# lordet01/SE_SNMF_NAT

Measured on AMD Instinct MI355X. Metric: NMF multiplicative-update iterations/sec (FxTxr), higher is better.
Workload: dtype f32; 1 GPU; single-MI355X sparse NMF basis train (BASELINE configs[1]): 257x100000 frames, r=256, KL, sparsity=5.0, full W+H update + objective per step; F=257, T=100000, r=256, beta=1, settle_steps=150

## Files before the change

### se_snmf_nat_amd/csrc/snmf_internal.h

```cpp
#pragma once
#include "snmf_kernels.h"

#include <algorithm>
#include <cmath>
#include <cstdarg>
#include <cstdio>
#include <cstring>
#include <deque>
#include <map>
#include <mutex>
#include <string>
#include <vector>

#include "snmf.h"

using namespace snmf;

extern thread_local std::string g_err;
int fail(int code, const char* fmt, ...);
#define HIP_TRY(expr)                                                                              \
    do {                                                                                           \
        hipError_t e_ = (expr);                                                                    \
        if (e_ != hipSuccess)                                                                      \
            return fail(e_ == hipErrorOutOfMemory ? SNMF_ERR_NOMEM : SNMF_ERR_NO_DEVICE, "%s: %s", \
// ... 82 lines not shown
    int NKT = 8, NWB = 4, WPS = 2, NLW = 0;
    int nbw = 2;
    int n_fg = 1, n_kg = 1, n_chunks = 1;
    static constexpr int stagger_w = 0;
    bool sf = false;
    int sf_grid = 1;
    bool wsf = false;
    size_t lds_wsf = 0;
    bool isf_share = false;
    bool wsf_share = false;
    bool isf = false;
    size_t lds_isf = 0;
    static constexpr int sf_stagger = 8000;
    size_t lds_sf = 0;
    int sf_share = 0, sf_nfull = 0;
    bool sr = false, wsr = false;
    int sr_grid = 1;
    static constexpr int sr_stagger = 1300;
    size_t lds_sr = 0, lds_wsr = 0;
    int til = 1;
    int n_ch1 = 0;
    bool wxg_off = false;
    bool wxg = false;
    int kq_chunks = 0, kq_kg = 0;
    size_t kq_lds = 0;
    size_t lds_w = 0;
    bool wfin = false;
    int wfin_S = 1;
    size_t lds_wfin = 0;
    bool fold_obj = false;
    bool gram_p = false;
    int gram_chunks = 0;
    bool generic = false;
    int frame_fb = 0, frame_kb = 0;
    size_t lds_frame = 0;
    size_t lds_mdi = 0;
    int grid_mdi = 1;
    bool small = false;
    bool small_ok = false;
    size_t lds_small = 0;
};
int plan_geometry(const snmf_params* p, int n_cu, PlanGeometry* g);
void describe_geometry(const PlanGeometry& g, const snmf_params& p, int n_cu, bool mdi, char* buf, size_t n);

struct snmf_plan : PlanGeometry {
    snmf_ctx* ctx = nullptr;
// ... 117 lines not shown
```

### se_snmf_nat_amd/csrc/snmf_kernels.h

```cpp
#pragma once
#include <hip/hip_runtime.h>
#include <stdint.h>

namespace snmf {

typedef float f32x2 __attribute__((ext_vector_type(2)));

typedef float f32x16 __attribute__((ext_vector_type(16)));
typedef float f32x4 __attribute__((ext_vector_type(4)));

constexpr float kFlr = 1e-9f;
constexpr int kMaxNW = 12;

constexpr int BM_GEN = 0;
constexpr int BM_KL = 1;
constexpr int BM_EUC = 2;

__device__ __forceinline__ f32x16 mfma32(float a, float b, f32x16 c) {
    return __builtin_amdgcn_mfma_f32_32x32x2f32(a, b, c, 0, 0, 0);
}
__device__ __forceinline__ f32x16 zero16() {
    f32x16 z;
#pragma unroll
    for (int i = 0; i < 16; ++i) z[i] = 0.f;
// ... 321 lines not shown
        wA[0] = ldw(q + 4);
        wA[1] = ldw(q + 5);
        sA[0] = *reinterpret_cast<const f32x4*>(bp + 32);
        sA[1] = *reinterpret_cast<const f32x4*>(bp + 40);
        bp += 32;
        SNMF_PIN();
        mmstage(wB, sB);
    }
    if (q < nq) {
#pragma unroll
        for (int e = 0; e < 4; ++e) acc = mfma32(sA[0][e], wA[0][e], acc);
    }
    if (q + 1 < nq) {
#pragma unroll
        for (int e = 0; e < 4; ++e) acc = mfma32(sA[1][e], wA[1][e], acc);
    }
    if (q + 2 < nq) {
        const f32x4 w2 = ldw(q + 2);
        const f32x4 s2 = *reinterpret_cast<const f32x4*>(bp + 16);
#pragma unroll
        for (int e = 0; e < 4; ++e) acc = mfma32(s2[e], w2[e], acc);
    }
}

__device__ __forceinline__ void stagger_start(int cycles, unsigned linear_block, unsigned n_blocks, int shift) {
    const bool late = shift >= 0 ? ((linear_block >> shift) & 1u) != 0 : linear_block >= n_blocks / 2;
    if (cycles > 0 && late) {
        const unsigned long long t0 = __builtin_amdgcn_s_memtime();
        while (__builtin_amdgcn_s_memtime() - t0 < (unsigned long long)cycles) __builtin_amdgcn_s_sleep(32);
    }
}

template <int NTHREADS>
__device__ __forceinline__ void stage_in(const float* __restrict__ src, float* dst, int cols, int rowlen, int ld,
                                         int tid) {
    const int r4 = rowlen / 4;
    const int n4 = cols * r4;
    constexpr int B = 8;
    for (int i0 = tid; i0 < n4; i0 += B * NTHREADS) {
        f32x4 x[B];
#pragma unroll
        for (int b = 0; b < B; ++b) {
            const int i = i0 + b * NTHREADS;
            if (i < n4) x[b] = *reinterpret_cast<const f32x4*>(src + 4 * (size_t)i);
        }
        SNMF_PIN();
// ... 2359 lines not shown
            dps[k] = k < sa.Rx ? 0.f : hw;
        }
        __builtin_amdgcn_wave_barrier();
        for (int part = 0; part < 2; ++part) {
            hsolve_frame_p1<FB, KB>(wr, part ? dps : sps, wxs, lamp, xlam, Fm, xr, kb, fb, lane);
            __syncthreads();
            for (int f = tid; f < Fm && f < F; f += NTHR) {
                float s = lamp[f];
#pragma unroll
                for (int q = 1; q < 8; ++q) s += lamp[q * Fm + f];
                out[part * F + f] = s;
            }
            if (xr && tid == 0) {
                float s = xlam[0];
#pragma unroll
                for (int q = 1; q < 8; ++q) s += xlam[q];
                out[part * F + Fm] = s;
            }
            __syncthreads();
        }
    }
}

template <int NK, int NWB, int NL, int WPS, int WM, int BM, bool OBJ, int TT, int LX, bool TIL, bool XG = false>
__device__ __forceinline__ void wstats_body(StepArgs a, int n_chunks, int mat_index, int n_mat) {
    static_assert(TT == 32 || (TT == 16 && NL == 0), "narrow tiles: 16 frames, synchronous staging");
    static_assert(!XG || (WM != 3 && !TIL), "the extra row rides in P3's gate: needs a P3, every consumer on every tile");
    constexpr int NTHR = (NWB + NL) * 64;
    const int NBUF = NL > 0 ? (a.nbuf == 3 ? 3 : 2) : 1;
    if (a.stop && *a.stop) return;
    extern __shared__ __attribute__((aligned(16))) float lds[];
    const int ldv = 32 * NWB;
    constexpr bool LDHC = (NK == 4 || NK == 8) && TT == 32;
    const int ldh = LDHC ? (NK == 4 ? 132 : 260) : a.ldh;
    const int bufsz = TT * (ldh + ldv);
    float* wxs = lds + NBUF * bufsz;
    const int lane = threadIdx.x & 63, w = wave_index();
    const bool is_loader = NL > 0 && w >= NWB;
    const int fl = lane & 31, h = lane >> 5;
    const int rp = a.rp, Fp = a.Fp;
    int chunk = blockIdx.x, by = blockIdx.y, nch = n_chunks;
    if (a.n_ch1 > 0) {
        by = 0;
        if (chunk >= n_chunks) {
            const int c1 = chunk - n_chunks;
            by = 1 + c1 / a.n_ch1;
            chunk = c1 - (by - 1) * a.n_ch1;
            nch = a.n_ch1;
        }
    }
// ... 38 lines not shown
    const bool do_s = WM == 0 && by == 0 && blockIdx.z == 0;
    float ssum[4] = {0.f, 0.f, 0.f, 0.f};
    double acc_div = 0.0;

    static_assert(NL == 0 || (NL == 4 && (NWB == 4 || NWB == 8)), "progress slots: four per loader role, NWB consumers");
    unsigned* ready = reinterpret_cast<unsigned*>(wxs + rp);
    unsigned* done = ready + 4;
    float* vx = reinterpret_cast<float*>(done + NWB);
    float* gxs = wxs + rp + 128;
    const unsigned gxa = (unsigned)(uintptr_t)(__attribute__((address_space(3))) void*)(gxs + w * gxw + 4 * lane);
    const bool idle_c = NL > 0 && NWB == 4 && !is_loader && !active && !do_x;
    if (NL > 0) {
        if (threadIdx.x < 4 + NWB) ready[threadIdx.x] = 0u;
        __syncthreads();
        if constexpr (NWB == 4) {
            if (idle_c && lane == 0) done[w] = 0xffffffffu;
            __syncthreads();
        }
    }

    auto xrow_tile = [&](const float* xH, int xt0, int xw, const float* vxc) {
            float rxv[CPW];
            float dsum = 0.f;
#pragma unroll
            for (int c0 = 0; c0 < CPW; c0 += 4) {
                const int tl = xw * CPW + c0 + (lane >> 4);
                const int kl = lane & 15;
                const float* hrow = xH + tl * ldh;
                const int t = xt0 + tl;
                const float v = vxc[tl];
                float rv;
                if (WM != 3) {
                    float s0 = 0.f, s1 = 0.f;
                    for (int k = 4 * kl; k < rp; k += 64) {
                        const f32x4 wv = *reinterpret_cast<const f32x4*>(wxs + k);
                        const f32x4 hv = *reinterpret_cast<const f32x4*>(hrow + k);
                        s0 += wv[0] * hv[0] + wv[1] * hv[1];
                        s1 += wv[2] * hv[2] + wv[3] * hv[3];
                    }
                    const float s = row_sum_f(s0 + s1);
                    const float lam = fmaxf(s, kFlr);
                    if (OBJ && kl == 0) dsum += (t < a.T) ? div_term<BM>(v, lam, a.beta, a.inv_bb1) : 0.f;
                    if (WM == 0) rv = v * fast_rcp(lam);
                    else if (WM == 1) rv = den_of_lam<BM>(lam, a.beta);
                    else rv = v * numfac_of_lam<BM>(lam, a.beta);
                } else {
                    rv = v;
                }
#pragma unroll
                for (int c = 0; c < 4; ++c)
                    rxv[c0 + c] = __int_as_float(__builtin_amdgcn_readlane(__float_as_int(rv), 16 * c));
            }
            if (OBJ) acc_div += (double)dsum;
#pragma unroll
            for (int pc = 0; pc < NPC; ++pc) {
                const int k0 = 256 * pc + 4 * lane;
                if (k0 + (kc ? kap_base * 32 : 0) < rp) {
                    f32x4 g4;
                    if (GXL) asm volatile("ds_read_b128 %0, %1\n\ts_waitcnt lgkmcnt(0)" : "=v"(g4) : "v"(gxa));
#pragma unroll
                    for (int c = 0; c < CPW; ++c) {
                        const f32x4 hv = *reinterpret_cast<const f32x4*>(xH + (xw * CPW + c) * ldh + k0);
#pragma unroll
                        for (int e = 0; e < 4; ++e) {
                            if (GXL) g4[e] += rxv[c] * hv[e];
                            else gx[4 * pc + e] += rxv[c] * hv[e];
                        }
                    }
                    if (GXL) asm volatile("ds_write_b128 %0, %1" ::"v"(gxa), "v"(g4));
                }
            }
    };
    float rs4[NPC][4];
#pragma unroll
    for (int pp = 0; pp < NPC; ++pp)
#pragma unroll
        for (int e = 0; e < 4; ++e) rs4[pp][e] = 0.f;
    if (is_loader) {
        typedef __attribute__((address_space(3))) void* lds_ptr_t;
        const int lw = w - NWB;
        const int npc = (rp + 255) >> 8;
        const int nVb = TT * Fp * 4;
        const int c0 = by * NWB * 32;
        const int cw = (a.Fm - c0 < NWB * 32 ? a.Fm - c0 : NWB * 32);
        auto dma_tile = [&](int tile, float* dst, int bi) {
            const __amdgpu_buffer_rsrc_t rh =
                __builtin_amdgcn_make_buffer_rsrc(const_cast<float*>(a.Hin + (size_t)tile * TT * rp), 0, TT * rp * 4, 0x00020000);
            const int pc0 = kc ? (int)blockIdx.z : 0, pcn = kc ? 1 : npc;
            for (int t = lw; t < TT; t += NL)
                for (int pc = 0; pc < pcn; ++pc)
                    if ((pc0 + pc) * 256 + lane * 4 < rp)
                        __builtin_amdgcn_raw_ptr_buffer_load_lds(rh, (lds_ptr_t)(dst + t * ldh + pc * 256), 16, lane * 16,
                                                                 (t * rp + (pc0 + pc) * 256) * 4, 0, 0);
            const __amdgpu_buffer_rsrc_t rv =
                __builtin_amdgcn_make_buffer_rsrc(const_cast<float*>(a.V + (size_t)tile * TT * Fp), 0, nVb, 0x00020000);
            for (int t = lw; t < TT; t += NL)
                for (int pc = 0; pc * 256 < cw; ++pc)
                    if (pc * 256 + lane * 4 < cw)
                        __builtin_amdgcn_raw_ptr_buffer_load_lds(rv, (lds_ptr_t)(dst + TT * ldh + t * ldv + pc * 256), 16, lane * 16,
                                                                 (t * Fp + c0 + pc * 256) * 4, 0, 0);
            if (do_x && lw == 0 && lane < TT)
                __builtin_amdgcn_raw_ptr_buffer_load_lds(rv, (lds_ptr_t)(vx + bi * 32), 4, lane * Fp * 4, a.Fm * 4, 0, 0);
        };
        auto sums_of = [&](const float* H) {
            if (!do_s) return;
            for (int t = lw; t < TT; t += NL)
#pragma unroll
                for (int pc = 0; pc < NPC; ++pc)
                    if (pc < npc && pc * 256 + lane * 4 < rp) {
                        const f32x4 hv = *reinterpret_cast<const f32x4*>(H + t * ldh + pc * 256 + lane * 4);
#pragma unroll
                        for (int e = 0; e < 4; ++e) rs4[pc][e] += hv[e];
                    }
        };
        if (tb < te) {
            dma_tile(tb, lds, 0);
            asm volatile("s_waitcnt vmcnt(0)" ::: "memory");
            sums_of(lds);
            rp_post(ready, lw, 1u, lane);
        }
        int nb = 0;
        for (int tile = tb, it = 0; tile + 1 < te; ++tile, ++it) {
            nb = nb + 1 == NBUF ? 0 : nb + 1;
            float* nH = lds + nb * bufsz;
            if (it + 2 - NBUF > 0) {
                rp_await(done, (unsigned)(it + 2 - NBUF), a.stop);
                if (NWB == 8) rp_await(done + 4, (unsigned)(it + 2 - NBUF), a.stop);
            }
            dma_tile(tile + 1, nH, nb);
            asm volatile("s_waitcnt vmcnt(0)" ::: "memory");
            sums_of(nH);
            rp_post(ready, lw, (unsigned)(it + 2), lane);
        }
    }

    if (NL > 0 && NWB == 8 && !is_loader && w >= 4 && a.stagger > 0 && tb < te) {
        const unsigned long long ts = __builtin_amdgcn_s_memtime();
        while (__builtin_amdgcn_s_memtime() - ts < (unsigned long long)a.stagger) __builtin_amdgcn_s_sleep(16);
    }
    SNMF_STAMP_DECL
    int cb = NL > 0 ? NBUF - 1 : 0;
    int te_c = te;
    if constexpr (NWB == 4) {
        if (idle_c) te_c = tb;
    }
    for (int tile = tb, it = 0; tile < te_c && !is_loader; ++tile, ++it) {
        const int t0 = tile * TT;
        SNMF_STAMP(0);
        if (NL > 0) cb = cb + 1 == NBUF ? 0 : cb + 1;
        float* Hs = lds + cb * bufsz;
        float* Vs = Hs + TT * ldh;
        if (NL == 0) {
            __syncthreads();
            stage_in<NST>(a.Hin + (size_t)t0 * rp, Hs, TT, rp, ldh, sid);
            {
                const int c0 = by * NWB * 32, cw4 = (a.Fm - c0 < NWB * 32 ? a.Fm - c0 : NWB * 32) / 4, n4 = TT * cw4;
                const float* vsrc = a.V + (size_t)t0 * Fp + c0;
                constexpr int B = 8;
                for (int i0 = sid; i0 < n4; i0 += B * NST) {
                    f32x4 x[B];
#pragma unroll
                    for (int b = 0; b < B; ++b) {
                        const int i = i0 + b * NST;
                        if (i < n4) x[b] = *reinterpret_cast<const f32x4*>(vsrc + (size_t)(i / cw4) * Fp + 4 * (i % cw4));
                    }
#pragma unroll
                    for (int b = 0; b < B; ++b) {
                        const int i = i0 + b * NST;
                        if (i < n4) *reinterpret_cast<f32x4*>(Vs + (i / cw4) * ldv + 4 * (i % cw4)) = x[b];
                    }
                }
                if (do_x && sid < TT) vx[sid] = a.V[(size_t)(t0 + sid) * Fp + a.Fm];
            }
            __syncthreads();
        }
        if (NL > 0) rp_await(ready, (unsigned)(it + 1), a.stop);
        SNMF_STAMP(1);
        if (NL == 0 && do_s) {
#pragma unroll
            for (int j = 0; j < 4; ++j) {
                const int k = sid + j * NST;
                if (k < rp) {
                    float sacc = 0.f;
                    for (int t = 0; t < TT; ++t) sacc += Hs[t * ldh + k];
                    ssum[j] += sacc;
                }
            }
        }
        if (!XG && do_x) xrow_tile(Hs, t0, w, vx + cb * 32);
        SNMF_STAMP(2);
        if (!active || (TIL && til > 1 && it % til != tph)) {
            if constexpr (XG) {
                if (do_x) xrow_tile(Hs, t0, w, vx + cb * 32);
            }
            if (NL > 0) rp_post(done, w, (unsigned)(it + 1), lane);
            continue;
        }

        float R[16];
        if (WM != 3) {
            f32x16 acc1[1] = {zero16()};
            const f32x4* wp = reinterpret_cast<const f32x4*>(a.Wt4 + (size_t)phi * rp * 32) + lane;
            {
                const __amdgpu_buffer_rsrc_t rsw = wimage_rsrc(a.Wt4, (size_t)a.nf * rp * 32);
                const float* spl = Hs + (fl & (TT - 1)) * ldh + 4 * h;
                if constexpr (XG) {
                    auto xgate = [&]() {
                        if (do_x) xrow_tile(Hs, t0, w, vx + cb * 32);
                    };
                    if (a.nqk == 32) contract_p3_buf<true>(acc1[0], rsw, lane * 16, phi * rp * 128, spl, 32, xgate);
                    else contract_p3_buf<false>(acc1[0], rsw, lane * 16, phi * rp * 128, spl, a.nqk, xgate);
                } else {
                    if (a.nqk == 32) contract_p3_buf<true>(acc1[0], rsw, lane * 16, phi * rp * 128, spl, 32, NoGate());
                    else contract_p3_buf<false>(acc1[0], rsw, lane * 16, phi * rp * 128, spl, a.nqk, NoGate());
                }
            }
            SNMF_STAMP(3);
            const f32x16 acc = acc1[0];
            const int f = phi * 32 + fl;
            float dsum = 0.f;
            auto ratio_rows = [&](auto masked) {
#pragma unroll
                for (int i = 0; i < 16; ++i) {
                    if (TT < 32 && i >= TT / 2) {
                        R[i] = 0.f;
                        continue;
                    }
                    const int t = t0 + drow(i, h);
                    const float v = Vs[drow(i, h) * ldv + fc];
                    float lam = fmaxf(acc[i], kFlr);
                    if (OBJ) {
                        if (do_obj) {
                            float d = div_term<BM>(v, lam, a.beta, a.inv_bb1);
                            if (decltype(masked)::value) {
                                dsum += (f < a.F && t < a.T) ? d : 0.f;
                            } else {
#pragma clang fp contract(off)
                                dsum = dsum + d;
                            }
                        }
                    }
                    if (WM == 0) R[i] = v * fast_rcp(lam);
                    else if (WM == 1) R[i] = den_of_lam<BM>(lam, a.beta);
                    else R[i] = v * numfac_of_lam<BM>(lam, a.beta);
                }
            };
            if (OBJ && TT == 32 && phi * 32 + 32 <= a.F && t0 + 32 <= a.T) ratio_rows(std::false_type{});
            else ratio_rows(std::true_type{});
            if (OBJ) acc_div += (double)dsum;
        } else {
            const int f = phi * 32 + fl;
#pragma unroll
            for (int i = 0; i < 16; ++i) R[i] = (TT < 32 && i >= TT / 2) ? 0.f : Vs[drow(i, h) * ldv + fc];
        }
        SNMF_STAMP(4);
        const float* hb = Hs + (4 * h) * ldh + fl + (kc ? 0 : kap_base * 32);
        const float* hrow[16];
#pragma unroll
        for (int i = 0; i < 16; ++i) hrow[i] = hb + ((i & 3) + 8 * (i >> 2)) * ldh;
        float b0[16], b1[16];
        auto ldb = [&](float (&b)[16], int kap) {
#pragma unroll
            for (int i = 0; i < TT / 2; ++i) b[i] = hrow[i][kap * 32];
        };
#define SNMF_KTILE(KP, CUR, NXT)                                                  \
    if constexpr ((KP) < NK) {                                                    \
        if (kap_base + (KP) < nkm) {  \
            if constexpr ((KP) + 1 < NK) ldb(NXT, (KP) + 1);                      \
            SNMF_PIN();                                                           \
            _Pragma("unroll") for (int i = 0; i < TT / 2; ++i) G[KP] = mfma32(R[i], CUR[i], G[KP]); \
        }                                                                         \
    }
        ldb(b0, 0);
        SNMF_KTILE(0, b0, b1)
        SNMF_KTILE(1, b1, b0)
        SNMF_KTILE(2, b0, b1)
        SNMF_KTILE(3, b1, b0)
        SNMF_KTILE(4, b0, b1)
        SNMF_KTILE(5, b1, b0)
        SNMF_KTILE(6, b0, b1)
        SNMF_KTILE(7, b1, b0)
        SNMF_KTILE(8, b0, b1)
        SNMF_KTILE(9, b1, b0)
        SNMF_KTILE(10, b0, b1)
        SNMF_KTILE(11, b1, b0)
        SNMF_KTILE(12, b0, b1)
        SNMF_KTILE(13, b1, b0)
        SNMF_KTILE(14, b0, b1)
        SNMF_KTILE(15, b1, b0)
#undef SNMF_KTILE
        if constexpr (LX > 0) {
            const int koff = (a.nk - 1) * 32 - fl;
#pragma unroll
            for (int i0 = 0; i0 < TT / 2; i0 += 4) {
#pragma unroll
                for (int i = i0; i < i0 + 4; ++i) {
                    const f32x4 h0 = *reinterpret_cast<const f32x4*>(hrow[i] + koff);
#pragma unroll
                    for (int e = 0; e < 4; ++e) gl[e] += R[i] * h0[e];
                }
                if constexpr (LX > 1) {
#pragma unroll
                    for (int i = i0; i < i0 + 4; ++i) {
                        const f32x4 h1 = *reinterpret_cast<const f32x4*>(hrow[i] + koff + 4);
#pragma unroll
                        for (int e = 0; e < 4; ++e) gl[4 + e] += R[i] * h1[e];
                    }
                }
                SNMF_PIN();
            }
        }
        if (NL > 0) rp_post(done, w, (unsigned)(it + 1), lane);
        SNMF_STAMP(5);
    }
#ifdef SNMF_PROF
    if (!is_loader && a.prof) {
        const size_t wv = ((size_t)(blockIdx.x + gridDim.x * blockIdx.y)) * NWB + w;
        if (wv < 4096) {
            SNMF_STAMP_OUT(a.prof + (4096 + wv) * 12, 12);
            SNMF_STAMP_CLK(a.prof, 4096 + wv);
        }
    }
#endif

    if constexpr (TIL && NL > 0) if (til > 1) {
        float* xs = lds;
        constexpr int NV = NK * 16 + (LX ? 4 * LX : 0);
        __syncthreads();
        if (active && tph > 0) {
            float* dst = xs + (size_t)((tph - 1) * nfl + wl) * NV * 64 + lane;
#pragma unroll
            for (int k = 0; k < NK; ++k)
#pragma unroll
                for (int i = 0; i < 16; ++i) dst[(k * 16 + i) * 64] = G[k][i];
            if constexpr (LX > 0) {
// ... 97 lines not shown
        double* red = reinterpret_cast<double*>(lds);
        red[threadIdx.x] = acc_div;
        __syncthreads();
        constexpr int P2 = NTHR >= 512 ? 512 : 256;
        if ((int)threadIdx.x + P2 < NTHR) red[threadIdx.x] += red[threadIdx.x + P2];
        __syncthreads();
        for (int s = P2 / 2; s > 0; s >>= 1) {
            if ((int)threadIdx.x < s) red[threadIdx.x] += red[threadIdx.x + s];
            __syncthreads();
        }
        if (threadIdx.x == 0 && blockIdx.z == 0) {
            const int slot = a.n_ch1 > 0 ? (int)blockIdx.x : by * n_chunks + chunk;
            a.part[2 * slot] = red[0];
            a.part[2 * slot + 1] = 0.0;
        }
    }
}

template <int NK, int NWB, int NL, int WPS, int WM, int BM, bool OBJ, int TT = 32, int LX = 0>
__global__ __launch_bounds__((NWB + NL) * 64, WPS) void k_wstats(StepArgs a, int n_chunks, int mat_index,
                                                                 int n_mat) {
    wstats_body<NK, NWB, NL, WPS, WM, BM, OBJ, TT, LX, false>(a, n_chunks, mat_index, n_mat);
}
template <int NK, int NWB, int NL, int WPS, int WM, int BM, bool OBJ>
__global__ __launch_bounds__((NWB + NL) * 64, WPS) void k_wstats_xg(StepArgs a, int n_chunks, int mat_index, int n_mat) {
    wstats_body<NK, NWB, NL, WPS, WM, BM, OBJ, 32, 0, false, true>(a, n_chunks, mat_index, n_mat);
}
template <int NK, int NWB, int NL, int WPS, int WM, int BM, bool OBJ, int TT = 32, int LX = 0>
__global__ __launch_bounds__((NWB + NL) * 64, WPS) void k_wstats_teams(StepArgs a, int n_chunks, int mat_index,
                                                                       int n_mat) {
    wstats_body<NK, NWB, NL, WPS, WM, BM, OBJ, TT, LX, true>(a, n_chunks, mat_index, n_mat);
}


struct ReduceArgs {
    const float* slabs;
    const float* spart;
    const double* part;
    double* stats;
    const int* stop;
    int n_chunks, n_mat, n_part, rp, Fp;
    double* qp_buf;
    unsigned* fin_cnt;
    int r;
    int do_mats;
    int do_obj;
    double sh_const;
    int use_sh_const;
    int check_it;
// ... 682 lines not shown
```

### se_snmf_nat_amd/csrc/snmf_tu_geometry.hip

```cpp
#include "snmf_internal.h"
#include "snmf_generic.h"

namespace {
struct Switches {
    bool hstep_rp;
    bool hstep_split;
    bool wstats_nl;
    bool wstats_xg;
    bool iter_sf;
    bool gram_p;
    int no_small;
    bool hfold;
};
int env_int(const char* name, int unset) {
    const char* e = getenv(name);
    return e ? atoi(e) : unset;
}
Switches read_switches() {
    Switches s;
    s.hstep_rp = env_int("SNMF_HSTEP_RP", 1) != 0;
    s.hstep_split = env_int("SNMF_HSTEP_SPLIT", 1) != 0;
    s.wstats_nl = env_int("SNMF_WSTATS_NL", 4) == 4;
    s.wstats_xg = env_int("SNMF_WSTATS_XG", 1) != 0;
    s.iter_sf = env_int("SNMF_ITER_SF", 1) != 0;
    s.gram_p = env_int("SNMF_GRAM_P", 1) != 0;
    s.no_small = env_int("SNMF_NO_SMALL", 0);
    s.hfold = env_int("SNMF_HFOLD", 1) != 0;
    return s;
}
}

int plan_geometry(const snmf_params* pp, int n_cu, PlanGeometry* g) {
    SN_TRY(validate_params(pp));
    const snmf_params& p = *pp;
    const Switches sw = read_switches();
    *g = PlanGeometry{};
    const int F = p.F, T = p.T, r = p.r;
    int n_h = 0, n_w = 0;
    for (int k = 0; k < r; ++k) {
        n_h += p.h_update_ind ? p.h_update_ind[k] != 0 : 1;
        n_w += p.w_update_ind ? p.w_update_ind[k] != 0 : 1;
    }
    if (n_h != 0 && n_h != r)
        return fail(SNMF_ERR_DIM, "partial h_update_ind (%d of %d rows): dimension mismatch in src/sparse_nmf.m:192/197/202", n_h, r);
    g->upd_h = n_h > 0;
    g->upd_w = n_w > 0;
// ... 154 lines not shown
    const int wg_w = g->NLW ? 1 : g->WPS;
    g->n_chunks = std::max(1, std::min(n_tiles_w, n_cu * wg_w / std::max(1, g->n_fg * g->n_kg)));
    g->n_ch1 = 0;
    if (g->xr && g->n_fg >= 2 && g->n_kg == 1 && g->NLW && g->upd_w && n_tiles_w >= 4 * g->n_chunks) {
        const int tot = g->n_fg * g->n_chunks, ng1 = g->n_fg - 1;
        const double x = (600.0 + 6.0 * g->rp) / (82.0 * (g->rp / 2 + 16 * g->nk)) * 4.0 / g->NWB;
        auto n1_of = [&](int n0) { return (tot - n0) / ng1; };
        auto cost = [&](int n0) {
            return std::max(std::ceil((double)n_tiles_w / n0) * (1.0 + x), std::ceil((double)n_tiles_w / n1_of(n0)));
        };
        int best = g->n_chunks;
        for (int n0 = g->n_chunks + 1; n0 <= g->n_chunks + g->n_chunks / 4 && n1_of(n0) >= 1; ++n0)
            if (cost(n0) < cost(best) - 1e-9) best = n0;
        if (best != g->n_chunks) {
            g->n_ch1 = n1_of(best);
            g->n_chunks = best;
        }
    }
    {
        const bool shape = g->xr && g->bm == BM_KL && g->upd_w && g->upd_h && g->NKT == 8 && g->NWB == 4 && g->NLW == 4 && g->TTW == 32 &&
                           g->n_fg <= 2 && g->n_kg == 1 && !g->wsr;
        g->wxg = shape && sw.wstats_xg;
        g->wxg_off = shape && !sw.wstats_xg;
    }
    {
        const int mf_h = (g->nf + g->NWH - 1) / g->NWH * g->NT * (g->rp / 2) +
                         (g->nk + g->NWH - 1) / g->NWH * g->NT * (g->Fq / 2);
        g->stagger_h = (g->grid_h > n_cu) ? mf_h * 64 : 0;
    }
    if (g->lds_w > lds_cap && g->upd_w) g->generic = true;
    if (g->bm == BM_EUC && g->NKT == 16 && g->TTW == 32 && g->upd_w) {
        g->kq_kg = (g->nk + 7) / 8;
        g->kq_chunks = std::max(1, std::min(std::min(n_tiles_w, g->n_chunks), n_cu / std::max(1, g->n_fg * g->kq_kg)));
        g->kq_lds = (size_t)2 * 32 * (260 + 32 * 4) * 4 + (size_t)g->rp * 4 + 512 + (size_t)4 * 256 * 4;
    }
    if (g->bm == BM_EUC && g->upd_w && g->upd_h && g->TTW == 32 && r < 2 * F && sw.gram_p) {
        g->gram_p = true;
        const int nfg_g = (g->rp / 32 + g->NWB - 1) / g->NWB;
        g->gram_chunks = g->kq_kg ? g->kq_chunks
                                    : std::max(1, std::min(n_tiles_w, n_cu * (g->NLW ? 1 : g->WPS) / std::max(1, nfg_g)));
    }
    if (g->rp > 4 * g->NWB * 64 && g->upd_w && (g->bm == BM_KL || g->xr)) g->generic = true;

    g->lds_wfin = (size_t)9 * g->n_mat * g->Fp * sizeof(double);
    g->wfin = g->upd_w && g->lds_wfin + 12 * 1024 <= lds_cap;
    {
// ... 9 lines not shown
        g->lds_small = need;
        if (g->small_ok && sw.no_small == 0) {
            static const int fbs[2] = {4, 8}, kbs[2] = {16, 25};
            for (int fi = 0; fi < 2 && !g->frame_fb; ++fi)
                for (int ki = 0; ki < 2 && !g->frame_fb; ++ki)
                    if (F <= 64 * fbs[fi] + 1 && r <= 8 * kbs[ki]) {
                        g->frame_fb = fbs[fi];
                        g->frame_kb = kbs[ki];
                    }
            if (g->frame_fb) {
                const int Fm2 = 64 * g->frame_fb, RB = 8 * g->frame_kb, nv = g->bm == BM_KL ? 1 : 2;
                g->lds_frame = (size_t)(40 + 4 * RB + 3 * (Fm2 + 4) + 8 * Fm2 + nv * 16 * (RB + 1)) * 4;
                if (g->lds_frame > lds_cap) g->frame_fb = g->frame_kb = 0;
            }
        }
    }
    if (g->generic) {
        g->hstep_rp = g->rh = false;
        g->rh_lxh = 0;
        g->rp_S = 0;
        g->kq_kg = 0;
        g->gram_p = false;
        g->n_ch1 = 0;
        g->wxg = g->wxg_off = false;
        g->small_ok = g->small = false;
        g->frame_fb = g->frame_kb = 0;
        g->wfin = false;
        g->n_fg = g->n_kg = 1;
        g->n_chunks = (T + kGChunkT - 1) / kGChunkT;
        g->grid_h = g->grid_mdi = kGBlocks;
    }
    g->fold_obj = g->upd_h && !g->upd_w && !g->generic && sw.hfold;
    g->isf = g->isf && g->wfin && g->n_chunks == g->sf_grid;
    g->isf_share = g->isf && sw.hstep_split;
    if (!g->upd_h || g->generic) g->hupd = HUPD_PLAIN;
    else if (g->sr) g->hupd = HUPD_SR;
    else if (g->sf) g->hupd = HUPD_SF;
    else if (g->rh) g->hupd = HUPD_RH;
    else if (g->NWH == 8 && g->NLH == 4 && g->hstep_rp && g->bm == BM_KL) g->hupd = HUPD_RP;
    else g->hupd = HUPD_PLAIN;
    return SNMF_OK;
}

void describe_geometry(const PlanGeometry& g, const snmf_params& p, int n_cu, bool mdi, char* buf, size_t n) {
    if (g.generic) {
        snprintf(buf, n, "F=%d T=%d r=%d beta=%g | out-of-envelope path (intermediates in HBM: k_g_gemm / k_g_ratio / k_g_hupd, %d frame splits) | n_cu=%d",
                 p.F, p.T, p.r, p.beta, g.n_chunks, n_cu);
// ... 14 lines not shown
    case HUPD_RH:
        snprintf(hs, sizeof hs, "k_hstep_rh (4 P1 + 4 P2 + 4 loader waves on half tiles%s; %d of %d tiles pipelined, last round split %d ways, grid %d)",
                 g.rh_lxh == 1 ? ", P2 cut four ways over the contraction + leftover columns as 4x4x1 MFMAs" : (g.rh_lxh == 2 ? ", P2 in wave pairs cut over the contraction + leftover columns as 4x4x1 MFMAs" : ""), g.rp_full, g.rp_tiles, g.rp_S, g.rp_grid);
        break;
    case HUPD_RP:
        snprintf(hs, sizeof hs, "k_hstep_rp (4 P1 + 4 P2 + 4 loader waves%s; %d of %d tiles pipelined, last round split %d ways, grid %d)",
                 g.rp_cut == 2 ? ", P2 in wave pairs cut over the contraction" : g.rp_cut ? ", P2 cut four ways over the contraction" : "", g.rp_full, g.rp_tiles, g.rp_S, g.rp_grid);
        break;
    case HUPD_PLAIN:
        if (mdi)
            snprintf(hs, sizeof hs, "k_hstep (MDI pass: 8 waves on 32-frame tiles, synchronous staging, V re-imputed in place; %d tiles)", g.Tp / 32);
        else
            snprintf(hs, sizeof hs, "k_hstep");
        break;
    }
    const int grid = mdi ? g.grid_mdi : h == HUPD_SR ? g.sr_grid : h == HUPD_SF ? g.sf_grid : (h == HUPD_RH || h == HUPD_RP) ? g.rp_grid : g.grid_h;
    const int threads = (mdi || h == HUPD_SR || h == HUPD_SF) ? 512 : h == HUPD_RH ? 768 : (g.NWH + g.NLH) * 64;
    const size_t lds = mdi ? g.lds_mdi : h == HUPD_SR ? g.lds_sr : h == HUPD_SF ? g.lds_sf : h == HUPD_RH ? g.lds_rh : g.lds_h;
    const char* wkind = g.gram_p ? ", P = W*(H*H') through the Gram matrix"
                        : g.wsr  ? ", k_wstats_sr: statistics rows per wave, operands straight into the MFMA layouts"
                        : g.wsf  ? (g.wsf_share ? ", k_wstats_sf: a tile per wave, a single remainder tile shared by the eight waves" : ", k_wstats_sf: a tile per wave")
                        : g.til > 1 ? (g.til == 2 ? ", 2 consumer teams take the tiles in turn" : ", 4+ consumer teams take the tiles in turn")
                        : g.wxg_off ? ", extra row at the top of the tile (SNMF_WSTATS_XG=0)"
                                    : "";
    const char* wfinish = g.wfin    ? "k_wfin"
                          : g.upd_w ? "k_reduce + k_wapply"
                          : (g.fold_obj && !mdi) ? "none (objective fold + convergence test on the H step's last workgroup)"
                                                 : "none (objective fold + convergence test: k_reduce)";
    snprintf(buf, n,
             "F=%d T=%d r=%d beta=%g | Fm=%d(+%d VALU row) rp=%d Tp=%d | hstep: %s, tile=%d frames, grid=%d x %d thr, lds=%zu B | "
             "wstats: NK=%d waves=%d+%d grid=(%d chunks,%d fgroups,%d kgroups; group-1 chunks %d) lds=%zu B%s | W finish (run loop): %s | n_cu=%d",
             p.F, p.T, p.r, p.beta, g.Fm, g.xr, g.rp, g.Tp, hs, mdi ? 32 : g.TTH * g.NT, grid, threads, lds, g.NKT, g.NWB, g.NLW, g.n_chunks, g.n_fg,
             g.n_kg, g.n_ch1 ? g.n_ch1 : g.n_chunks, g.lds_w, wkind, wfinish, n_cu);
}

extern "C" int snmf_plan_geometry_describe(const snmf_params* p, int32_t n_cu, char* buf, size_t buflen) {
    if (!buf) return fail(SNMF_ERR_INVALID, "NULL argument");
    if (n_cu <= 0) return fail(SNMF_ERR_INVALID, "n_cu must be positive (got %d)", (int)n_cu);
    PlanGeometry g;
    SN_TRY(plan_geometry(p, n_cu, &g));
    describe_geometry(g, *p, n_cu, false, buf, buflen);
    return SNMF_OK;
}
```

### se_snmf_nat_amd/csrc/snmf_wstats_dispatch.h

```cpp
#pragma once
#include "snmf_internal.h"
#include "snmf_generic.h"

template <int NK, int NWB, int NL, int WPS, int WM, int BM, bool OBJ, int TT = 32, int LX = 0, bool TIL = false>
static int launch_wstats_one(snmf_plan* pl, const StepArgs& a, int mat_index) {
    if constexpr (!TIL && NK == 4 && NL > 0 && WM == 0 && BM == BM_KL && TT == 32) {
        if (pl->til > 1) return launch_wstats_one<NK, NWB, NL, WPS, WM, BM, OBJ, TT, LX, true>(pl, a, mat_index);
    }
    const bool split = pl->n_ch1 > 0;
    dim3 g(split ? pl->n_chunks + (pl->n_fg - 1) * pl->n_ch1 : pl->n_chunks, split ? 1 : pl->n_fg, pl->n_kg), b((NWB + NL) * 64);
    StepArgs as = a;
    as.n_ch1 = split ? pl->n_ch1 : 0;
    if (!TIL) as.til = 1;
    if constexpr (TIL) {
        auto kern = k_wstats_teams<NK, NWB, NL, WPS, WM, BM, OBJ, TT, LX>;
        SN_TRY(ensure_dyn_lds(pl->ctx->device, (const void*)kern, pl->lds_w));
        hipLaunchKernelGGL(kern, g, b, pl->lds_w, pl->ctx->stream, as, pl->n_chunks, mat_index, pl->n_mat);
    } else {
        auto kern = k_wstats<NK, NWB, NL, WPS, WM, BM, OBJ, TT, LX>;
        SN_TRY(ensure_dyn_lds(pl->ctx->device, (const void*)kern, pl->lds_w));
        hipLaunchKernelGGL(kern, g, b, pl->lds_w, pl->ctx->stream, as, pl->n_chunks, mat_index, pl->n_mat);
    }
    HIP_TRY(hipGetLastError());
    return SNMF_OK;
// ... 20 lines not shown
    } else {
        auto kern = k_wstats<NK, NWB, NL, WPS, 3, BM_EUC, false, 32>;
        SN_TRY(ensure_dyn_lds(pl->ctx->device, (const void*)kern, pl->lds_w));
        hipLaunchKernelGGL(kern, dim3(pl->gram_chunks, (ag.nf + NWB - 1) / NWB, 1), dim3((NWB + NL) * 64), pl->lds_w, pl->ctx->stream, ag,
                           pl->gram_chunks, 0, 1);
    }
    HIP_TRY(hipGetLastError());
    const size_t n = (size_t)pl->rp * pl->rp;
    hipLaunchKernelGGL(k_gram_sum, dim3((int)std::min<size_t>((n + 255) / 256, 4096)), dim3(256), 0, pl->ctx->stream,
                       (const float*)pl->gram_slabs, pl->gram_chunks, n, pl->gram32, (const int*)&pl->st->stop);
    HIP_TRY(hipGetLastError());
    const int nsplit = std::max(1, std::min(std::min(8, pl->n_chunks), (pl->p.r + 31) / 32));
    const int kchunk = (((pl->p.r + nsplit - 1) / nsplit) + 15) / 16 * 16;
    const long long nW = (long long)pl->Fp * pl->rp;
    return g_gemm(pl, pl->Wcf, 1, pl->Fp, pl->gram32, 1, pl->rp, pl->slabs + nW, 1, pl->Fp, pl->p.F, pl->p.r, pl->p.r, kchunk,
                  nW * pl->n_mat);
}
template <int NK, int NWB, int NL, int WPS>
static int launch_wstats_xg(snmf_plan* pl, const StepArgs& a) {
    StepArgs as = a;
    const bool split = pl->n_ch1 > 0;
    as.n_ch1 = split ? pl->n_ch1 : 0;
    as.til = 1;
    auto kern = k_wstats_xg<NK, NWB, NL, WPS, 0, BM_KL, false>;
    SN_TRY(ensure_dyn_lds(pl->ctx->device, (const void*)kern, pl->lds_w));
    dim3 g(split ? pl->n_chunks + (pl->n_fg - 1) * pl->n_ch1 : pl->n_chunks, split ? 1 : pl->n_fg, 1);
    hipLaunchKernelGGL(kern, g, dim3((NWB + NL) * 64), pl->lds_w, pl->ctx->stream, as, pl->n_chunks, 0, pl->n_mat);
    HIP_TRY(hipGetLastError());
    return SNMF_OK;
}
template <int NK, int NWB, int NL, int WPS, int TT = 32>
static int launch_wstats_geo(snmf_plan* pl, const StepArgs& a, bool obj) {
    if (pl->bm == BM_KL) {
        if constexpr (NK == 8 && NWB == 4 && NL == 4 && TT == 32) {
            if (pl->wxg) {
                if (obj || pl->n_kg != 1) return fail(SNMF_ERR_INTERNAL, "k_wstats_xg: not the statistics of a full update");
                return launch_wstats_xg<NK, NWB, NL, WPS>(pl, a);
            }
        }
        const int left = pl->p.r - 32 * (pl->nk - 1);
        const int lx = (pl->nk >= 2 && pl->n_kg == 1 && left <= 8) ? (left + 3) / 4 : 0;
        if constexpr (NL > 0 && TT == 32 && NK == 4) {
            if (lx == 1) return obj ? launch_wstats_one<NK, NWB, NL, WPS, 0, BM_KL, true, TT, 1>(pl, a, 0)
                                    : launch_wstats_one<NK, NWB, NL, WPS, 0, BM_KL, false, TT, 1>(pl, a, 0);
            if constexpr (NWB == 4) {
                if (lx == 2) return obj ? launch_wstats_one<NK, NWB, NL, WPS, 0, BM_KL, true, TT, 2>(pl, a, 0)
                                        : launch_wstats_one<NK, NWB, NL, WPS, 0, BM_KL, false, TT, 2>(pl, a, 0);
// ... 31 lines not shown
```

Baseline: 2212 iterations/s.

## Add latency-hiding variant of extra-row W statistics kernel

Adds a LAT-templated variant of k_wstats_xg, enabled by default through SNMF_WSTATS_LAT. It preloads the first W fragments before the tile loop and prefetches V and H epilogue values inside the contraction's hook. It also issues wider per-lane DMA for H and V tiles, unrolls the extra-row dot products with early LDS reads, and polls the loader's ready flags ahead so the next wait can be skipped. The goal is to hide memory and LDS latency in the W-statistics pass, at the cost of more registers and more complex, geometry-specific code paths.

```diff
diff --git a/se_snmf_nat_amd/csrc/snmf_internal.h b/se_snmf_nat_amd/csrc/snmf_internal.h
--- a/se_snmf_nat_amd/csrc/snmf_internal.h
+++ b/se_snmf_nat_amd/csrc/snmf_internal.h
@@ -128,6 +128,8 @@
     int n_ch1 = 0;
     bool wxg_off = false;
     bool wxg = false;
+    bool wlat = false;
+    bool wlat_off = false;
     int kq_chunks = 0, kq_kg = 0;
     size_t kq_lds = 0;
     size_t lds_w = 0;
diff --git a/se_snmf_nat_amd/csrc/snmf_kernels.h b/se_snmf_nat_amd/csrc/snmf_kernels.h
--- a/se_snmf_nat_amd/csrc/snmf_kernels.h
+++ b/se_snmf_nat_amd/csrc/snmf_kernels.h
@@ -367,6 +367,95 @@
         for (int e = 0; e < 4; ++e) acc = mfma32(s2[e], w2[e], acc);
     }
 }
+template <bool UNROLL32, typename Gate, typename Pre>
+__device__ __forceinline__ void contract_p3_res(f32x16& acc, __amdgpu_buffer_rsrc_t rs, int voff, int soff0, const float* sp,
+                                                int nq, const f32x4 (&wR)[2], Gate gate, Pre pre) {
+    f32x4 wA[2], wB[2], sA[2], sB[2];
+    int sbase = soff0;
+    asm volatile("" : "+s"(sbase));
+    auto ldw = [&](int q) { return ldw_buf(rs, voff + (q & 3) * 1024, sbase + (q >> 2) * 4096); };
+    auto mmstage = [&](const f32x4 (&w)[2], const f32x4 (&sf)[2]) {
+#pragma unroll
+        for (int j = 0; j < 2; ++j)
+#pragma unroll
+            for (int e = 0; e < 4; ++e) acc = mfma32(sf[j][e], w[j][e], acc);
+    };
+    wB[0] = ldw(2);
+    wB[1] = ldw(3);
+    SNMF_PIN();
+    gate();
+    sA[0] = *reinterpret_cast<const f32x4*>(sp);
+    sA[1] = *reinterpret_cast<const f32x4*>(sp + 8);
+    if (UNROLL32) {
+#pragma unroll
+        for (int q = 0; q < 32; q += 4) {
+            if (q == 28) pre();
+            if (q > 0) {
+                wB[0] = ldw(q + 2);
+                wB[1] = ldw(q + 3);
+            }
+            sB[0] = *reinterpret_cast<const f32x4*>(sp + 8 * (q + 2));
+            sB[1] = *reinterpret_cast<const f32x4*>(sp + 8 * (q + 3));
+            SNMF_PIN();
+            if (q == 0) mmstage(wR, sA);
+            else mmstage(wA, sA);
+            wA[0] = ldw(q + 4);
+            wA[1] = ldw(q + 5);
+            sA[0] = *reinterpret_cast<const f32x4*>(sp + 8 * (q + 4));
+            sA[1] = *reinterpret_cast<const f32x4*>(sp + 8 * (q + 5));
+            SNMF_PIN();
+            mmstage(wB, sB);
+        }
+        return;
+    }
+    const float* bp = sp;
+    int q = 0;
+    auto four = [&](const f32x4 (&w0)[2], auto ldb_) {
+        if (decltype(ldb_)::value) {
+            wB[0] = ldw(q + 2);
+            wB[1] = ldw(q + 3);
+        }
+        sB[0] = *reinterpret_cast<const f32x4*>(bp + 16);
+        sB[1] = *reinterpret_cast<const f32x4*>(bp + 24);
+        SNMF_PIN();
+        mmstage(w0, sA);
+        wA[0] = ldw(q + 4);
+        wA[1] = ldw(q + 5);
+        sA[0] = *reinterpret_cast<const f32x4*>(bp + 32);
+        sA[1] = *reinterpret_cast<const f32x4*>(bp + 40);
+        bp += 32;
+        q += 4;
+        SNMF_PIN();
+        mmstage(wB, sB);
+    };
+    if (nq >= 8) {
+        four(wR, std::false_type{});
+        while (q + 7 < nq) four(wA, std::true_type{});
+        pre();
+        four(wA, std::true_type{});
+    } else if (nq >= 4) {
+        pre();
+        four(wR, std::false_type{});
+    } else {
+        pre();
+        wA[0] = wR[0];
+        wA[1] = wR[1];
+    }
+    if (q < nq) {
+#pragma unroll
+        for (int e = 0; e < 4; ++e) acc = mfma32(sA[0][e], wA[0][e], acc);
+    }
+    if (q + 1 < nq) {
+#pragma unroll
+        for (int e = 0; e < 4; ++e) acc = mfma32(sA[1][e], wA[1][e], acc);
+    }
+    if (q + 2 < nq) {
+        const f32x4 w2 = ldw(q + 2);
+        const f32x4 s2 = *reinterpret_cast<const f32x4*>(bp + 16);
+#pragma unroll
+        for (int e = 0; e < 4; ++e) acc = mfma32(s2[e], w2[e], acc);
+    }
+}
 
 __device__ __forceinline__ void stagger_start(int cycles, unsigned linear_block, unsigned n_blocks, int shift) {
     const bool late = shift >= 0 ? ((linear_block >> shift) & 1u) != 0 : linear_block >= n_blocks / 2;
@@ -2772,10 +2861,17 @@
     }
 }
 
-template <int NK, int NWB, int NL, int WPS, int WM, int BM, bool OBJ, int TT, int LX, bool TIL, bool XG = false>
+#ifndef SNMF_WSTATS_LAT_SET
+#define SNMF_WSTATS_LAT_SET 31
+#endif
+constexpr int kWstatsLat = SNMF_WSTATS_LAT_SET;
+template <int NK, int NWB, int NL, int WPS, int WM, int BM, bool OBJ, int TT, int LX, bool TIL, bool XG = false, int LAT = 0>
 __device__ __forceinline__ void wstats_body(StepArgs a, int n_chunks, int mat_index, int n_mat) {
     static_assert(TT == 32 || (TT == 16 && NL == 0), "narrow tiles: 16 frames, synchronous staging");
     static_assert(!XG || (WM != 3 && !TIL), "the extra row rides in P3's gate: needs a P3, every consumer on every tile");
+    static_assert(LAT == 0 || (XG && NL == 4 && NWB == 4 && TT == 32 && LX == 0), "LAT: k_wstats_xg's geometry");
+    static_assert((LAT & 2) == 0 || (LAT & 1) != 0, "LAT 2: the epilogue's reads ride on contract_p3_res's hook");
+    static_assert((LAT & 16) == 0 || (XG && NK <= 8), "LAT 16: the extra row's early reads assume one 256-column piece");
     constexpr int NTHR = (NWB + NL) * 64;
     const int NBUF = NL > 0 ? (a.nbuf == 3 ? 3 : 2) : 1;
     if (a.stop && *a.stop) return;
@@ -2860,6 +2956,15 @@
     auto xrow_tile = [&](const float* xH, int xt0, int xw, const float* vxc) {
             float rxv[CPW];
             float dsum = 0.f;
+            f32x4 g4e, hve[CPW];
+            if constexpr ((LAT & 16) != 0) {
+                if (4 * lane < rp) {
+                    g4e = *(const volatile __attribute__((address_space(3))) f32x4*)(uintptr_t)gxa;
+#pragma unroll
+                    for (int c = 0; c < CPW; ++c) hve[c] = *reinterpret_cast<const f32x4*>(xH + (xw * CPW + c) * ldh + 4 * lane);
+                }
+                SNMF_PIN();
+            }
 #pragma unroll
             for (int c0 = 0; c0 < CPW; c0 += 4) {
                 const int tl = xw * CPW + c0 + (lane >> 4);
@@ -2870,6 +2975,23 @@
                 float rv;
                 if (WM != 3) {
                     float s0 = 0.f, s1 = 0.f;
+                    if constexpr ((LAT & 16) != 0) {
+                        f32x4 wv4[4], hv4[4];
+#pragma unroll
+                        for (int j = 0; j < 4; ++j) {
+                            wv4[j] = *reinterpret_cast<const f32x4*>(wxs + 4 * kl + 64 * j);
+                            hv4[j] = *reinterpret_cast<const f32x4*>(hrow + 4 * kl + 64 * j);
+                        }
+#pragma unroll
+                        for (int j = 0; j < 4; ++j) {
+                            if (4 * kl + 64 * j < rp) {
+#pragma clang fp contract(off)
+                                const f32x4 wv = wv4[j], hv = hv4[j];
+                                s0 += wv[0] * hv[0] + wv[1] * hv[1];
+                                s1 += wv[2] * hv[2] + wv[3] * hv[3];
+                            }
+                        }
+                    } else
                     for (int k = 4 * kl; k < rp; k += 64) {
                         const f32x4 wv = *reinterpret_cast<const f32x4*>(wxs + k);
                         const f32x4 hv = *reinterpret_cast<const f32x4*>(hrow + k);
@@ -2888,6 +3010,7 @@
 #pragma unroll
                 for (int c = 0; c < 4; ++c)
                     rxv[c0 + c] = __int_as_float(__builtin_amdgcn_readlane(__float_as_int(rv), 16 * c));
+                if constexpr ((LAT & 16) != 0) SNMF_PIN();
             }
             if (OBJ) acc_div += (double)dsum;
 #pragma unroll
@@ -2895,10 +3018,11 @@
                 const int k0 = 256 * pc + 4 * lane;
                 if (k0 + (kc ? kap_base * 32 : 0) < rp) {
                     f32x4 g4;
-                    if (GXL) asm volatile("ds_read_b128 %0, %1\n\ts_waitcnt lgkmcnt(0)" : "=v"(g4) : "v"(gxa));
+                    if constexpr ((LAT & 16) != 0) g4 = g4e;
+                    else if (GXL) asm volatile("ds_read_b128 %0, %1\n\ts_waitcnt lgkmcnt(0)" : "=v"(g4) : "v"(gxa));
 #pragma unroll
                     for (int c = 0; c < CPW; ++c) {
-                        const f32x4 hv = *reinterpret_cast<const f32x4*>(xH + (xw * CPW + c) * ldh + k0);
+                        const f32x4 hv = (LAT & 16) != 0 ? hve[c] : *reinterpret_cast<const f32x4*>(xH + (xw * CPW + c) * ldh + k0);
 #pragma unroll
                         for (int e = 0; e < 4; ++e) {
                             if (GXL) g4[e] += rxv[c] * hv[e];
@@ -2921,10 +3045,19 @@
         const int nVb = TT * Fp * 4;
         const int c0 = by * NWB * 32;
         const int cw = (a.Fm - c0 < NWB * 32 ? a.Fm - c0 : NWB * 32);
+        const int vpair = (lane & 31) * 16 + (lane >> 5) * Fp * 4;
         auto dma_tile = [&](int tile, float* dst, int bi) {
             const __amdgpu_buffer_rsrc_t rh =
                 __builtin_amdgcn_make_buffer_rsrc(const_cast<float*>(a.Hin + (size_t)tile * TT * rp), 0, TT * rp * 4, 0x00020000);
             const int pc0 = kc ? (int)blockIdx.z : 0, pcn = kc ? 1 : npc;
+            if constexpr ((LAT & 8) != 0) {
+                if (lane * 4 < rp) {
+#pragma unroll
+                    for (int j = 0; j < TT / NL; ++j)
+                        __builtin_amdgcn_raw_ptr_buffer_load_lds(rh, (lds_ptr_t)(dst + (lw + NL * j) * ldh), 16, lane * 16,
+                                                                 (lw + NL * j) * rp * 4, 0, 0);
+                }
+            } else
             for (int t = lw; t < TT; t += NL)
                 for (int pc = 0; pc < pcn; ++pc)
                     if ((pc0 + pc) * 256 + lane * 4 < rp)
@@ -2932,6 +3065,12 @@
                                                                  (t * rp + (pc0 + pc) * 256) * 4, 0, 0);
             const __amdgpu_buffer_rsrc_t rv =
                 __builtin_amdgcn_make_buffer_rsrc(const_cast<float*>(a.V + (size_t)tile * TT * Fp), 0, nVb, 0x00020000);
+            if ((LAT & 8) != 0 && cw == 128) {
+#pragma unroll
+                for (int j = 0; j < TT / 2 / NL; ++j)
+                    __builtin_amdgcn_raw_ptr_buffer_load_lds(rv, (lds_ptr_t)(dst + TT * ldh + 2 * (lw + NL * j) * ldv), 16, vpair,
+                                                             (2 * (lw + NL * j) * Fp + c0) * 4, 0, 0);
+            } else
             for (int t = lw; t < TT; t += NL)
                 for (int pc = 0; pc * 256 < cw; ++pc)
                     if (pc * 256 + lane * 4 < cw)
@@ -2942,6 +3081,18 @@
         };
         auto sums_of = [&](const float* H) {
             if (!do_s) return;
+            if constexpr ((LAT & 8) != 0) {
+                if (lane * 4 < rp) {
+                    f32x4 hv[TT / NL];
+#pragma unroll
+                    for (int j = 0; j < TT / NL; ++j) hv[j] = *reinterpret_cast<const f32x4*>(H + (lw + NL * j) * ldh + lane * 4);
+#pragma unroll
+                    for (int j = 0; j < TT / NL; ++j)
+#pragma unroll
+                        for (int e = 0; e < 4; ++e) rs4[0][e] += hv[j][e];
+                }
+                return;
+            }
             for (int t = lw; t < TT; t += NL)
 #pragma unroll
                 for (int pc = 0; pc < NPC; ++pc)
@@ -2976,6 +3127,15 @@
         const unsigned long long ts = __builtin_amdgcn_s_memtime();
         while (__builtin_amdgcn_s_memtime() - ts < (unsigned long long)a.stagger) __builtin_amdgcn_s_sleep(16);
     }
+    f32x4 wres[2] = {{0.f, 0.f, 0.f, 0.f}, {0.f, 0.f, 0.f, 0.f}};
+    if constexpr ((LAT & 1) != 0) {
+        if (active) {
+            const __amdgpu_buffer_rsrc_t rsw = wimage_rsrc(a.Wt4, (size_t)a.nf * rp * 32);
+            wres[0] = ldw_buf(rsw, lane * 16, phi * rp * 128);
+            wres[1] = ldw_buf(rsw, lane * 16 + 1024, phi * rp * 128);
+        }
+    }
+    unsigned ahead = 0u;
     SNMF_STAMP_DECL
     int cb = NL > 0 ? NBUF - 1 : 0;
     int te_c = te;
@@ -3012,6 +3172,15 @@
             }
             __syncthreads();
         }
+        if constexpr ((LAT & 4) != 0) {
+            if (ahead >= (unsigned)(it + 1)) {
+                __builtin_amdgcn_fence(__ATOMIC_ACQUIRE, "workgroup", "local");
+                stress_jitter();
+            } else {
+                rp_await(ready, (unsigned)(it + 1), a.stop);
+            }
+            ahead = 0u;
+        } else
         if (NL > 0) rp_await(ready, (unsigned)(it + 1), a.stop);
         SNMF_STAMP(1);
         if (NL == 0 && do_s) {
@@ -3036,13 +3205,31 @@
         }
 
         float R[16];
+        float vpre[16], bpre[16];
         if (WM != 3) {
             f32x16 acc1[1] = {zero16()};
             const f32x4* wp = reinterpret_cast<const f32x4*>(a.Wt4 + (size_t)phi * rp * 32) + lane;
             {
                 const __amdgpu_buffer_rsrc_t rsw = wimage_rsrc(a.Wt4, (size_t)a.nf * rp * 32);
                 const float* spl = Hs + (fl & (TT - 1)) * ldh + 4 * h;
-                if constexpr (XG) {
+                if constexpr (XG && LAT != 0) {
+                    auto xgate = [&]() {
+                        if (do_x) xrow_tile(Hs, t0, w, vx + cb * 32);
+                    };
+                    auto vread = [&]() {
+                        if constexpr ((LAT & 2) != 0) {
+#pragma unroll
+                            for (int i = 0; i < 16; ++i) vpre[i] = Vs[drow(i, h) * ldv + fc];
+                        }
+                    };
+                    if constexpr ((LAT & 1) != 0) {
+                        if (a.nqk == 32) contract_p3_res<true>(acc1[0], rsw, lane * 16, phi * rp * 128, spl, 32, wres, xgate, vread);
+                        else contract_p3_res<false>(acc1[0], rsw, lane * 16, phi * rp * 128, spl, a.nqk, wres, xgate, vread);
+                    } else {
+                        if (a.nqk == 32) contract_p3_buf<true>(acc1[0], rsw, lane * 16, phi * rp * 128, spl, 32, xgate);
+                        else contract_p3_buf<false>(acc1[0], rsw, lane * 16, phi * rp * 128, spl, a.nqk, xgate);
+                    }
+                } else if constexpr (XG) {
                     auto xgate = [&]() {
                         if (do_x) xrow_tile(Hs, t0, w, vx + cb * 32);
                     };
@@ -3054,6 +3241,11 @@
                 }
             }
             SNMF_STAMP(3);
+            if constexpr ((LAT & 2) != 0) {
+#pragma unroll
+                for (int i = 0; i < 16; ++i) bpre[i] = Hs[(4 * h + (i & 3) + 8 * (i >> 2)) * ldh + fl + kap_base * 32];
+                SNMF_PIN();
+            }
             const f32x16 acc = acc1[0];
             const int f = phi * 32 + fl;
             float dsum = 0.f;
@@ -3065,7 +3257,7 @@
                         continue;
                     }
                     const int t = t0 + drow(i, h);
-                    const float v = Vs[drow(i, h) * ldv + fc];
+                    const float v = (LAT & 2) != 0 ? vpre[i] : Vs[drow(i, h) * ldv + fc];
                     float lam = fmaxf(acc[i], kFlr);
                     if (OBJ) {
                         if (do_obj) {
@@ -3102,6 +3294,7 @@
             for (int i = 0; i < TT / 2; ++i) b[i] = hrow[i][kap * 32];
         };
 #define SNMF_KTILE(KP, CUR, NXT)                                                  \
+    if constexpr ((LAT & 4) != 0 && (KP) == NK - 1) ready_ahead();                \
     if constexpr ((KP) < NK) {                                                    \
         if (kap_base + (KP) < nkm) {  \
             if constexpr ((KP) + 1 < NK) ldb(NXT, (KP) + 1);                      \
@@ -3109,7 +3302,19 @@
             _Pragma("unroll") for (int i = 0; i < TT / 2; ++i) G[KP] = mfma32(R[i], CUR[i], G[KP]); \
         }                                                                         \
     }
-        ldb(b0, 0);
+        unsigned ra[4] = {0u, 0u, 0u, 0u};
+        auto ready_ahead = [&]() {
+            if (tile + 1 < te_c) {
+#pragma unroll
+                for (int i = 0; i < 4; ++i) ra[i] = __hip_atomic_load(ready + i, __ATOMIC_RELAXED, __HIP_MEMORY_SCOPE_WORKGROUP);
+            }
+        };
+        if constexpr ((LAT & 2) != 0) {
+#pragma unroll
+            for (int i = 0; i < 16; ++i) b0[i] = bpre[i];
+        } else {
+            ldb(b0, 0);
+        }
         SNMF_KTILE(0, b0, b1)
         SNMF_KTILE(1, b1, b0)
         SNMF_KTILE(2, b0, b1)
@@ -3149,6 +3354,10 @@
             }
         }
         if (NL > 0) rp_post(done, w, (unsigned)(it + 1), lane);
+        if constexpr ((LAT & 4) != 0) {
+            const unsigned lo01 = ra[0] < ra[1] ? ra[0] : ra[1], lo23 = ra[2] < ra[3] ? ra[2] : ra[3];
+            ahead = (unsigned)__builtin_amdgcn_readfirstlane((int)(lo01 < lo23 ? lo01 : lo23));
+        }
         SNMF_STAMP(5);
     }
 #ifdef SNMF_PROF
@@ -3292,9 +3501,9 @@
                                                                  int n_mat) {
     wstats_body<NK, NWB, NL, WPS, WM, BM, OBJ, TT, LX, false>(a, n_chunks, mat_index, n_mat);
 }
-template <int NK, int NWB, int NL, int WPS, int WM, int BM, bool OBJ>
+template <int NK, int NWB, int NL, int WPS, int WM, int BM, bool OBJ, int LAT = 0>
 __global__ __launch_bounds__((NWB + NL) * 64, WPS) void k_wstats_xg(StepArgs a, int n_chunks, int mat_index, int n_mat) {
-    wstats_body<NK, NWB, NL, WPS, WM, BM, OBJ, 32, 0, false, true>(a, n_chunks, mat_index, n_mat);
+    wstats_body<NK, NWB, NL, WPS, WM, BM, OBJ, 32, 0, false, true, LAT>(a, n_chunks, mat_index, n_mat);
 }
 template <int NK, int NWB, int NL, int WPS, int WM, int BM, bool OBJ, int TT = 32, int LX = 0>
 __global__ __launch_bounds__((NWB + NL) * 64, WPS) void k_wstats_teams(StepArgs a, int n_chunks, int mat_index,
diff --git a/se_snmf_nat_amd/csrc/snmf_tu_geometry.hip b/se_snmf_nat_amd/csrc/snmf_tu_geometry.hip
--- a/se_snmf_nat_amd/csrc/snmf_tu_geometry.hip
+++ b/se_snmf_nat_amd/csrc/snmf_tu_geometry.hip
@@ -7,6 +7,7 @@
     bool hstep_split;
     bool wstats_nl;
     bool wstats_xg;
+    bool wstats_lat;
     bool iter_sf;
     bool gram_p;
     int no_small;
@@ -22,6 +23,7 @@
     s.hstep_split = env_int("SNMF_HSTEP_SPLIT", 1) != 0;
     s.wstats_nl = env_int("SNMF_WSTATS_NL", 4) == 4;
     s.wstats_xg = env_int("SNMF_WSTATS_XG", 1) != 0;
+    s.wstats_lat = env_int("SNMF_WSTATS_LAT", 1) != 0;
     s.iter_sf = env_int("SNMF_ITER_SF", 1) != 0;
     s.gram_p = env_int("SNMF_GRAM_P", 1) != 0;
     s.no_small = env_int("SNMF_NO_SMALL", 0);
@@ -222,6 +224,8 @@
                            g->n_fg <= 2 && g->n_kg == 1 && !g->wsr;
         g->wxg = shape && sw.wstats_xg;
         g->wxg_off = shape && !sw.wstats_xg;
+        g->wlat = g->wxg && sw.wstats_lat;
+        g->wlat_off = g->wxg && !sw.wstats_lat;
     }
     {
         const int mf_h = (g->nf + g->NWH - 1) / g->NWH * g->NT * (g->rp / 2) +
@@ -277,7 +281,7 @@
         g->kq_kg = 0;
         g->gram_p = false;
         g->n_ch1 = 0;
-        g->wxg = g->wxg_off = false;
+        g->wxg = g->wxg_off = g->wlat = g->wlat_off = false;
         g->small_ok = g->small = false;
         g->frame_fb = g->frame_kb = 0;
         g->wfin = false;
@@ -338,7 +342,8 @@
                         : g.wsf  ? (g.wsf_share ? ", k_wstats_sf: a tile per wave, a single remainder tile shared by the eight waves" : ", k_wstats_sf: a tile per wave")
                         : g.til > 1 ? (g.til == 2 ? ", 2 consumer teams take the tiles in turn" : ", 4+ consumer teams take the tiles in turn")
                         : g.wxg_off ? ", extra row at the top of the tile (SNMF_WSTATS_XG=0)"
-                                    : "";
+                        : g.wlat_off ? ", plain tile body (SNMF_WSTATS_LAT=0)"
+                                     : "";
     const char* wfinish = g.wfin    ? "k_wfin"
                           : g.upd_w ? "k_reduce + k_wapply"
                           : (g.fold_obj && !mdi) ? "none (objective fold + convergence test on the H step's last workgroup)"
diff --git a/se_snmf_nat_amd/csrc/snmf_wstats_dispatch.h b/se_snmf_nat_amd/csrc/snmf_wstats_dispatch.h
--- a/se_snmf_nat_amd/csrc/snmf_wstats_dispatch.h
+++ b/se_snmf_nat_amd/csrc/snmf_wstats_dispatch.h
@@ -66,7 +66,7 @@
     const bool split = pl->n_ch1 > 0;
     as.n_ch1 = split ? pl->n_ch1 : 0;
     as.til = 1;
-    auto kern = k_wstats_xg<NK, NWB, NL, WPS, 0, BM_KL, false>;
+    auto kern = pl->wlat ? k_wstats_xg<NK, NWB, NL, WPS, 0, BM_KL, false, kWstatsLat> : k_wstats_xg<NK, NWB, NL, WPS, 0, BM_KL, false>;
     SN_TRY(ensure_dyn_lds(pl->ctx->device, (const void*)kern, pl->lds_w));
     dim3 g(split ? pl->n_chunks + (pl->n_fg - 1) * pl->n_ch1 : pl->n_chunks, split ? 1 : pl->n_fg, 1);
     hipLaunchKernelGGL(kern, g, dim3((NWB + NL) * 64), pl->lds_w, pl->ctx->stream, as, pl->n_chunks, 0, pl->n_mat);
```

After: 2223 iterations/s, median of 6. Within noise of the previous version (+0.5%).
